# rlog58/dags-vae-search

Measured on AMD Instinct MI355X. Metric: DAGs/sec VAE+predictor train step, n=12 batch 4096 per GPU, at 1 MI355X, higher is better.
Workload: dtype f32 (fwd bf16x6, bwd bf16x3 split products, fp32 accumulate); 1 GPU; synthetic_v12 DAGs (n=12, card=12, N=15 tokens), PACE-VAE train step: pack + fwd + bwd + clip_grad_norm_(1.0) + Adam(1e-4), train mode dropout 0.15; per_gpu_batch=4096, global_batch=4096, waves_per_workgroup=8, parallelism=single

## Files before the change

### dags_vae_search_amd/csrc/dvs_api_backward.inc

```

static AttnBwdArgs attn_bwd_args(const Step& c, const DvsAttnP& ap, int block, int in, const DvsNormP* norm, const float* kv,
                                 const float* gpre, int site0) {
    AttnBwdArgs a;
    memset(&a, 0, sizeof(a));
    a.wimg = wimg_attn(c, block);
    a.dims = c.d;
    a.rec = c.rec;
    a.xin = c.ws + c.W.act[in];
    a.ln = ln_of(c, in, norm);
    a.kv = kv;
    a.in_w = c.P + ap.in_w;
    a.in_b = c.P + ap.in_b;
    a.out_w = c.P + ap.out_w;
    a.out_b = c.P + ap.out_b;
    a.gpre = gpre;
    a.gq = c.ws + c.W.gq;
    a.gk = c.ws + c.W.gk;
    a.gv = c.ws + c.W.gv;
    a.site_prob = site0;
    a.site_post = site0 + 1;
    a.slab = c.ws + c.W.slabs;
    a.P = c.L.total;
    a.o_out_w = ap.out_w;
    a.o_out_b = ap.out_b;
// ... 77 lines not shown
    const Step c = make_step(s, records, params, workspace, stream);
    if (int e = check_buffers(c, "dvs_loss_backward", records_bytes, n_params, workspace_bytes)) return e;
    const bool emit_loss = losses != nullptr;
    if (emit_loss && c.wide) return fail(13, "dvs_loss_backward_emit: one-tile path only (n_tokens, n_classes <= 16)");
    if (clip_scratch && 2 + dvs_sq_parts(c.L.total) > DVS_CLIP_SCRATCH_FLOATS)
        return fail(14, "dvs_loss_backward_sq: clip_scratch (DVS_CLIP_SCRATCH_FLOATS) is too small for this parameter count");
    call_begin();
    const DvsLayout& L = c.L;
    const DvsWorkspace& W = c.W;
    float* ws = c.ws;
    dvs_stream_t st = c.st;
    const bool wide = c.wide;
    const int grid = c.slabs;
    const int nw = c.nw;
    const bool chain = !wide && !split_stack();
    const bool chain_local = wide && !split_stack();
    BwdStackArgs stack;
    memset(&stack, 0, sizeof(stack));
    int stack_tag = 0;
    auto flush_stack = [&]() {
        if (stack.nphase > 0) dvs_launch_bwd_stack(stack, stack_tag, grid, nw, st);
        stack.nphase = 0;
        stack.has_latent = 0;
    };
    auto next_phase = [&](int kind) -> BwdPhase& {
        if (stack.nphase == DVS_STACK_PHASES) flush_stack();
        BwdPhase& ph = stack.ph[stack.nphase++];
        ph.kind = kind;
        return ph;
    };
    auto launch_ffn_bwd = [&](const FfnBwdArgs& f) {
        if (chain || chain_local) next_phase(DVS_PH_FFN).u.f = f;
        else dvs_launch_ffn_bwd(f, grid, nw, st);
    };
    auto launch_attn_bwd = [&](const AttnBwdArgs& a) {
        if (chain) {
            next_phase(DVS_PH_ATTN).u.a = a;
        } else if (wide) {
            flush_stack();
            dvs_launch_attn_bwd_w(a, grid, st);
        } else {
            dvs_launch_attn_bwd(a, grid, nw, st);
        }
    };
    auto launch_proj_bwd = [&](const ProjBwdArgs& a) {
        if (chain || chain_local) next_phase(DVS_PH_PROJ1 + 2).u.p = a;
        else dvs_launch_proj_bwd(a, 3, grid, nw, st);
    };

    float* cur = ws + W.gA;
    float* oth = ws + W.gB;
    {
        LossArgs la = loss_args(c);
        la.gcoef = gcoef;
        la.gout = cur;
        la.slab = ws + W.slabs;
        la.P = L.total;
        la.o_node0_w = L.node0_w;
        la.o_node0_b = L.node0_b;
        la.o_node2_w = L.node2_w;
        la.o_node2_b = L.node2_b;
        la.o_edge0_w = L.edge0_w;
        la.o_edge0_b = L.edge0_b;
        la.o_edge2_w = L.edge2_w;
        la.o_edge2_b = L.edge2_b;
        la.o_ln_g = L.dec[DVS_LAYERS - 1].n3.w;
        la.o_ln_b = L.dec[DVS_LAYERS - 1].n3.b;
        if (wide) dvs_launch_loss_bwd_w(la, grid, st);
        else dvs_launch_loss_bwd(la, grid, emit_loss, st);
        if (emit_loss) dvs_launch_finalize(finalize_args(c, status, losses, host_tail, host_seq), st);
    }
    const int dec_in = c.d.drop.on ? 7 : 0;
    for (int i = DVS_LAYERS - 1; i >= 0; --i) {
        const auto& pl = L.dec[i];
        const int s0 = slot_dec(i, 0), s1 = slot_dec(i, 1);
        launch_ffn_bwd(ffn_bwd_args(c, pl.ff, blk_dec_ffn(i), s1, pl.n2, cur, oth, site_dec(i, 4)));
        std::swap(cur, oth);
        launch_attn_bwd(attn_bwd_args(c, pl.ca, blk_dec_cross(i), s0, &pl.n1, ws + W.mem, cur, site_dec(i, 2)));
        ProjBwdArgs pq = proj_bwd_args(c, pl.ca, blk_dec_cross(i), s0, &pl.n1, cur, oth);
        pq.xin2 = ws + W.mem;
        pq.gout2 = ws + W.gmem;
        pq.accumulate_out2 = i != DVS_LAYERS - 1;
        launch_proj_bwd(pq);
        std::swap(cur, oth);
        const int sp = i > 0 ? slot_dec(i - 1, 2) : dec_in;
        const DvsNormP* np = i > 0 ? &L.dec[i - 1].n3 : nullptr;
        launch_attn_bwd(attn_bwd_args(c, pl.sa, blk_dec_self(i), sp, np, nullptr, cur, site_dec(i, 0)));
        launch_proj_bwd(proj_bwd_args(c, pl.sa, blk_dec_self(i), sp, np, cur, oth));
        std::swap(cur, oth);
    }
    flush_stack();
    stack_tag = 1;
    float* gdec_emb = cur;
    float* freebuf = oth;

    const bool fc_deferred = latent_in_chain(chain, nw);
    FcDwArgs fcdw;
    {
        LatentBwdArgs a;
        memset(&a, 0, sizeof(a));
        a.dims = c.d;
        a.gmem = ws + W.gmem;
        a.mu = ws + W.mu;
        a.logvar = ws + W.logvar;
        a.epsv = ws + W.epsv;
        a.limg = ws + W.limg;
        a.gcoef = gcoef;
        a.gz = ws + W.gz;
        a.genc = ws + W.genc;
        if (fc_deferred) {
            stack.has_latent = 1;
            stack.lat = a;
        } else {
            dvs_launch_latent_bwd(a, st);
        }
        FcDwArgs& f = fcdw;
        memset(&f, 0, sizeof(f));
        f.dims = c.d;
        f.gz = ws + W.gz;
        f.xenc = ws + W.enc_out;
        f.gmem = ws + W.gmem;
        f.z = ws + W.z;
        f.fcpart = ws + W.fcpart;
        f.P = L.total;
        f.o_fc1_w = L.fc1_w;
        f.o_fc1_b = L.fc1_b;
        f.o_fc2_w = L.fc2_w;
        f.o_fc2_b = L.fc2_b;
        f.o_fc3_w = L.fc3_w;
        f.o_fc3_b = L.fc3_b;
        if (!fc_deferred) dvs_launch_fc_dw(f, st);
    }
    cur = ws + W.genc;
    oth = freebuf;
    for (int i = DVS_LAYERS - 1; i >= 0; --i) {
        const auto& pl = L.enc[i];
        const int s0 = slot_enc(i, 0), s1 = slot_enc(i, 1);
        FfnBwdArgs f = ffn_bwd_args(c, pl.ff, blk_enc_ffn(i), s0, pl.n1, cur, oth, site_enc(i, 2));
        if (i == DVS_LAYERS - 1) {
            f.own_pre = ws + W.act[s1];
            f.own = ln_of(c, s1, &pl.n2);
            f.o_own_g = pl.n2.w;
            f.o_own_b = pl.n2.b;
        }
        launch_ffn_bwd(f);
        std::swap(cur, oth);
        const int sp = i > 0 ? slot_enc(i - 1, 1) : 0;
        const DvsNormP* np = i > 0 ? &L.enc[i - 1].n2 : nullptr;
        launch_attn_bwd(attn_bwd_args(c, pl.sa, blk_enc_attn(i), sp, np, nullptr, cur, site_enc(i, 0)));
        launch_proj_bwd(proj_bwd_args(c, pl.sa, blk_enc_attn(i), sp, np, cur, oth));
        std::swap(cur, oth);
    }
    flush_stack();
    if (fc_deferred) dvs_launch_fc_dw(fcdw, st);
    {
        EmbedArgs e = embed_args(c, 0);
        e.gout = cur;
        e.slab = ws + W.slabs;
        e.P = L.total;
        e.oW1 = L.W1;
        e.oW2 = L.W2;
        e.olab_w = L.lab_w;
        e.olab_b = L.lab_b;
        if (wide) dvs_launch_embed_bwd_w(e, gdec_emb, 2, grid, st);
        else dvs_launch_embed_bwd(e, gdec_emb, 2, grid, nw, st);
    }
    ReduceArgs r;
    r.slab = ws + W.slabs;
    r.fcpart = ws + W.fcpart;
    r.grads = grads;
    r.P = L.total;
    r.nslab = grid;
    r.fc_lo1 = L.fc1_w;
    r.fc_hi1 = L.dec[0].sa.in_w;
    r.fc_lo2 = L.fc3_w;
    r.fc_hi2 = L.total;
    r.sqpart = clip_scratch ? clip_scratch + 2 : nullptr;
    dvs_launch_reduce_slabs(r, st);
    return call_end("dvs_loss_backward");
}

extern "C" int dvs_clip_adam(int64_t n, float* params, float* grads, float* exp_avg, float* exp_avg_sq, float lr,
                             float beta1, float beta2, float adam_eps, int64_t step, float max_norm, float* scratch,
                             const float* guard, void* stream) {
    if (n <= 0 || !params || !grads || !exp_avg || !exp_avg_sq || !scratch) return fail(10, "dvs_clip_adam: bad argument");
    if (step < 1) return fail(12, "dvs_clip_adam: step is 1-based");
    call_begin();
    dvs_launch_clip_adam(n, params, grads, exp_avg, exp_avg_sq, lr, beta1, beta2, adam_eps, step, max_norm, scratch, guard, false,
                         (dvs_stream_t)stream);
    return call_end("dvs_clip_adam");
}

extern "C" int dvs_clip_adam_from_partials(int64_t n, float* params, float* grads, float* exp_avg, float* exp_avg_sq, float lr,
                                           float beta1, float beta2, float adam_eps, int64_t step, float max_norm,
                                           float* scratch, const float* guard, void* stream) {
    if (n <= 0 || !params || !grads || !exp_avg || !exp_avg_sq || !scratch) return fail(10, "dvs_clip_adam_from_partials: bad argument");
    if (step < 1) return fail(12, "dvs_clip_adam_from_partials: step is 1-based");
    if (2 + dvs_sq_parts(n) > DVS_CLIP_SCRATCH_FLOATS) return fail(14, "dvs_clip_adam_from_partials: more partials than the scratch holds");
    call_begin();
    dvs_launch_clip_adam(n, params, grads, exp_avg, exp_avg_sq, lr, beta1, beta2, adam_eps, step, max_norm, scratch, guard, true,
                         (dvs_stream_t)stream);
    return call_end("dvs_clip_adam_from_partials");
}
```

### dags_vae_search_amd/csrc/dvs_backward.h

```cpp
#pragma once
#include "dvs_kernels.h"
#include "dvs_stage.h"

struct FfnBwdArgs {
    DvsDims dims;
    const float* xin;
    DvsLN ln;
    const float *l1_w, *l1_b, *l2_w, *l2_b;
    const void* wimg;
    const float* gpre;
    const float* own_pre;
    DvsLN own;
    float* gout;
    int site_hidden, site_post;
    float* slab;
    int64_t P;
    int64_t o_l1_w, o_l1_b, o_l2_w, o_l2_b, o_ln_g, o_ln_b, o_own_g, o_own_b;
};

struct ProjBwdArgs {
    DvsDims dims;
    const float* xin;
    DvsLN ln;
    const float* w;
    const void* wimg;
    const float* gy[3];
    const float* gres;
    float* gout;
    int accumulate_out;
    int slot_order;
    const float* xin2;
    float* gout2;
    int accumulate_out2;
    float* slab;
    int64_t P;
    int64_t o_w, o_b, o_ln_g, o_ln_b;
};

struct AttnBwdArgs {
    DvsDims dims;
    const DvsRecord* rec;
    const float* xin;
    DvsLN ln;
    const float* kv;
    const float *in_w, *in_b, *out_w, *out_b;
    const void* wimg;
    const float* gpre;
    float *gq, *gk, *gv;
    int site_prob, site_post;
    float* slab;
    int64_t P;
    int64_t o_out_w, o_out_b;
    const float* qkv;
};

struct LatentBwdArgs {
    DvsDims dims;
    const float* gmem;
    const float *mu, *logvar, *epsv;
    const float* limg;
    const float* gcoef;
    float* gz;
    float* genc;
};

struct FcDwArgs {
    DvsDims dims;
    const float* gz;
    const float* xenc;
    const float* gmem;
    const float* z;
    float* fcpart;
    int64_t P;
    int64_t o_fc1_w, o_fc1_b, o_fc2_w, o_fc2_b, o_fc3_w, o_fc3_b;
};

struct ReduceArgs {
    const float* slab;
    const float* fcpart;
    float* grads;
    int64_t P;
    int nslab;
    int64_t fc_lo1, fc_hi1, fc_lo2, fc_hi2;
    float* sqpart;
};

enum { DVS_PH_FFN = 0, DVS_PH_ATTN = 1, DVS_PH_PROJ1 = 2, DVS_PH_PROJ2 = 3, DVS_PH_PROJ3 = 4 };
#define DVS_STACK_PHASES 9
struct BwdPhase {
    int kind, pad;
    union {
        FfnBwdArgs f;
        AttnBwdArgs a;
        ProjBwdArgs p;
    } u;
};
struct BwdStackArgs {
    int nphase;
    int has_latent;
    BwdPhase ph[DVS_STACK_PHASES];
    DvsStagePlan plan[DVS_STACK_PHASES];
    LatentBwdArgs lat;
};
static_assert(sizeof(BwdStackArgs) <= 4096, "kernel argument block limit");
void dvs_launch_bwd_stack(const BwdStackArgs& s, int tag, int grid, int nw, dvs_stream_t st);
void dvs_launch_ffn_bwd(const FfnBwdArgs& a, int grid, int nw, dvs_stream_t st);
void dvs_launch_proj_bwd(const ProjBwdArgs& a, int nproj, int grid, int nw, dvs_stream_t st);
void dvs_launch_attn_bwd(const AttnBwdArgs& a, int grid, int nw, dvs_stream_t st);
void dvs_launch_loss_bwd(const LossArgs& a, int grid, bool emit_loss, dvs_stream_t st);
void dvs_launch_embed_bwd(const EmbedArgs& a, const float* gout2, int site2, int grid, int nw, dvs_stream_t st);
void dvs_launch_latent_bwd(const LatentBwdArgs& a, dvs_stream_t st);
void dvs_launch_fc_dw(const FcDwArgs& a, dvs_stream_t st);
void dvs_launch_reduce_slabs(const ReduceArgs& a, dvs_stream_t st);
void dvs_launch_clip_adam(int64_t n, float* params, float* grads, float* m, float* v, float lr, float b1, float b2,
                          float eps, int64_t step, float max_norm, float* scratch, const float* guard, bool have_partials,
                          dvs_stream_t st);
inline int dvs_sq_parts(int64_t n) { return (int)(((n + 3) / 4 + 63) / 64); }

template <int OT, int IT>
__device__ __forceinline__ void dvs_stage_dw(float* region, const f4 (&dw)[OT][IT], const Lane& L) {
    constexpr int COLS = 16 * IT;
    float* mine = region + L.wave * (256 * OT * IT);
#pragma unroll
    for (int ot = 0; ot < OT; ++ot)
#pragma unroll
        for (int it = 0; it < IT; ++it)
#pragma unroll
            for (int reg = 0; reg < 4; ++reg) mine[(16 * ot + 4 * L.g + reg) * COLS + 16 * it + L.r] = dw[ot][it][reg];
}
template <int OT, int IT>
__device__ __forceinline__ void dvs_flush_dw(const float* region, float* dst, const Lane& L, int rows = 16 * OT,
                                             int ld_dst = 16 * IT, int cols_used = 16 * IT, bool rperm = false,
                                             bool cperm = false) {
    constexpr int COLS = 16 * IT, SZ = 256 * OT * IT;
    if (cperm) {
        for (int i = dvs_tid(); i < rows * COLS; i += blockDim.x) {
            float s = region[i];
            for (int w = 1; w < L.nwaves; ++w) s += region[w * SZ + i];
            const int row = i / COLS, col = i - row * COLS;
            dst[(size_t)(rperm ? dvs_pi(row) : row) * ld_dst + (cperm ? dvs_pi(col) : col)] = s;
        }
        return;
    }
    if (cols_used == COLS && (ld_dst & 3) == 0) {
        for (int i = dvs_tid() * 4; i < rows * COLS; i += blockDim.x * 4) {
            f4 s = *(const f4*)(region + i);
            for (int w = 1; w < L.nwaves; ++w) s += *(const f4*)(region + w * SZ + i);
            const int row = i / COLS, col = i - row * COLS;
            *(f4*)(dst + (size_t)(rperm ? dvs_pi(row) : row) * ld_dst + col) = s;
        }
        return;
    }
    for (int i = dvs_tid(); i < rows * COLS; i += blockDim.x) {
        float s = region[i];
        for (int w = 1; w < L.nwaves; ++w) s += region[w * SZ + i];
        const int row = i / COLS, col = i - row * COLS;
        if (col < cols_used) dst[(size_t)row * ld_dst + col] = s;
    }
}
template <int NT>
__device__ __forceinline__ void dvs_stage_vec(float* region, const f4 (&v)[NT], float* scr, const Lane& L) {
#pragma unroll
    for (int t = 0; t < NT; ++t) *(f4*)(scr + L.r * DVS_LD + 16 * t + 4 * L.g) = v[t];
    dvs_wave_sync();
    if (L.lane < 16 * NT) {
        float s = 0.f;
#pragma unroll
        for (int rr = 0; rr < 16; ++rr) s += scr[rr * DVS_LD + L.lane];
        region[L.wave * (16 * NT) + L.lane] = s;
    }
    dvs_wave_sync();
}
template <int NT>
__device__ __forceinline__ void dvs_flush_vec(const float* region, float* dst, const Lane& L, int n = 16 * NT,
                                              bool perm = false) {
    for (int i = dvs_tid(); i < n; i += blockDim.x) {
        float s = region[i];
        for (int w = 1; w < L.nwaves; ++w) s += region[w * (16 * NT) + i];
        dst[perm ? dvs_pi(i) : i] = s;
    }
}
constexpr int DVS_RED_MAT = 4 * 4096;
constexpr int DVS_RED_VEC = 4 * 64;

__device__ __forceinline__ void dvs_ln_bwd(f4 (&dx)[4], const f4 (&xhat)[4], float rstd, const float* lg, f4 (&dgam)[4],
                                           f4 (&dbet)[4], const Lane& L) {
    float s1 = 0.f, s2 = 0.f;
#pragma unroll
    for (int t = 0; t < 4; ++t) {
        const f4 g = dvs_vecT(lg, t, L);
#pragma unroll
        for (int kk = 0; kk < 4; ++kk) {
            dgam[t][kk] += dx[t][kk] * xhat[t][kk];
            dbet[t][kk] += dx[t][kk];
            const float dxh = dx[t][kk] * g[kk];
            dx[t][kk] = dxh;
            s1 += dxh;
            s2 += dxh * xhat[t][kk];
        }
    }
    s1 = dvs_sum_g(s1) * (1.f / 64.f);
    s2 = dvs_sum_g(s2) * (1.f / 64.f);
#pragma unroll
    for (int t = 0; t < 4; ++t)
#pragma unroll
        for (int kk = 0; kk < 4; ++kk) dx[t][kk] = rstd * (dx[t][kk] - s1 - xhat[t][kk] * s2);
}

struct DvsGroup {
    int* counter;
    int target;
};
__device__ __forceinline__ void dvs_group_barrier(DvsGroup& G, const Lane& L) {
    G.target += 4;
#ifdef DVS_EMU
    if (L.lane == 0) atomicAdd(G.counter, 1);
    while (__atomic_load_n(G.counter, __ATOMIC_RELAXED) < G.target) emu::yield();
    (void)emu::exchange(0, 0);
#else
    __builtin_amdgcn_fence(__ATOMIC_RELEASE, "workgroup");
    if (L.lane == 0) atomicAdd(G.counter, 1);
    for (int spins = 0; __hip_atomic_load(G.counter, __ATOMIC_RELAXED, __HIP_MEMORY_SCOPE_WORKGROUP) < G.target &&
                        spins < (1 << 24); ++spins)
        __builtin_amdgcn_s_sleep(1);
    __builtin_amdgcn_fence(__ATOMIC_ACQUIRE, "workgroup");
#endif
}
__device__ __forceinline__ void dvs_park_T(float* slot, const f4 (&v)[4], const Lane& L) {
#pragma unroll
    for (int t = 0; t < 4; ++t) *(f4*)(slot + L.r * DVS_LD + 16 * t + 4 * L.g) = v[t];
}
__device__ __forceinline__ float dvs_colsum(const float* slot, const Lane& L) {
    float s = 0.f;
#pragma unroll
    for (int rr = 0; rr < 16; ++rr) s += slot[rr * DVS_LD + L.lane];
    return s;
}
template <int NW = 8>
__device__ __forceinline__ void dvs_coop_stage(float* buf, const f4 (&acc)[4], const Lane& L) {
    if (NW == 4 || L.wave >= 4) return;
    const int ot = L.wave & 3;
#pragma unroll
    for (int it = 0; it < 4; ++it)
#pragma unroll
        for (int reg = 0; reg < 4; ++reg) buf[(16 * ot + 4 * L.g + reg) * 64 + 16 * it + L.r] = acc[it][reg];
}
template <int NW = 8>
__device__ __forceinline__ void dvs_coop_flush(const float* buf, float* dst, const f4 (&acc)[4], const Lane& L, bool rperm = false,
                                               bool cperm = false, int ld_dst = 64) {
    if (NW == 8 && L.wave < 4) return;
    const int ot = L.wave & 3;
#pragma unroll
    for (int it = 0; it < 4; ++it)
#pragma unroll
        for (int reg = 0; reg < 4; ++reg) {
            const int row = 16 * ot + 4 * L.g + reg, col = 16 * it + L.r;
            const float v = NW == 8 ? acc[it][reg] + buf[row * 64 + col] : acc[it][reg];
            dst[(size_t)(rperm ? dvs_pi(row) : row) * ld_dst + (cperm ? dvs_pi(col) : col)] = v;
        }
}
__device__ __forceinline__ void dvs_ln_bwd_core(f4 (&dx)[4], const f4 (&xhat)[4], float rstd, const float* lg, const Lane& L) {
    float s1 = 0.f, s2 = 0.f;
#pragma unroll
    for (int t = 0; t < 4; ++t) {
        const f4 g = dvs_vecT(lg, t, L);
// ... 24 lines not shown
```

### dags_vae_search_amd/csrc/k_backward_heads.hip

```cpp
#include "dvs_backward.h"
#include "dvs_wimg.h"
#include "dvs_latent_bwd.h"
#include "dvs_loss.h"

#ifdef DVS_STAMPS
__device__ unsigned long long dvs_stamps_lossb[256 * 4 * 12];
DVS_STAMP_READER(lossb)
#endif
#define LBSTAMP(k) DVS_ACC_STAMP_AT(dvs_stamps_lossb, lst_, 4, 12, k)
template <bool EMIT>
__global__ __launch_bounds__(256) void k_loss_bwd(LossArgs a, DvsStagePlan plan) {
#ifdef DVS_STAMPS
    unsigned long long lst_ = __builtin_amdgcn_s_memtime();
#endif
    DVS_DYN_LDS(smem);
    const LossLds l = loss_lds(smem);
    const int N = a.dims.N, C = a.dims.C;
    dvs_stage_now<(LOSS_CHUNKS + 3) / 4>(&plan, smem);
    __syncthreads();
    const Lane L = dvs_lane();
    float* scrV = l.scr + L.wave * 3 * DVS_SCR;
    float* scrU = scrV + DVS_SCR;
    float* dlm = scrU + DVS_SCR;
    const float b2 = l.b2[0];
// ... 108 lines not shown
            dvs_matb3<4>(V, hs, l.Wb, 64, 0, L);
        }
#pragma unroll
        for (int t = 0; t < 4; ++t) {
            *(f4*)(scrV + L.r * DVS_LD + 16 * t + 4 * L.g) = V[t];
            *(f4*)(scrU + L.r * DVS_LD + 16 * t + 4 * L.g) = U[t];
        }
        dvs_wave_sync();
        const unsigned par = rec->parents[(L.r + 1) & 15];
        LBSTAMP(3);
        f4 sU[4] = {f4_zero(), f4_zero(), f4_zero(), f4_zero()}, sV[4] = {f4_zero(), f4_zero(), f4_zero(), f4_zero()};
        for (int j0 = 0; j0 < N - 2; j0 += 2) {
            f4 pre[2][4], ev[2] = {f4_zero(), f4_zero()};
            const bool has2 = j0 + 1 < N - 2;
            const int jj[2] = {j0, has2 ? j0 + 1 : j0};
#pragma unroll
            for (int u = 0; u < 2; ++u)
#pragma unroll
                for (int t = 0; t < 4; ++t) {
                    const f4 x = U[t] + *(const f4*)(scrV + jj[u] * DVS_LD + 16 * t + 4 * L.g);
#pragma unroll
                    for (int kk = 0; kk < 4; ++kk) pre[u][t][kk] = fmaxf(x[kk], 0.f);
                    ev[u] += w2v[t] * pre[u][t];
                }
            float dl[2];
#pragma unroll
            for (int u = 0; u < 2; ++u) {
                const float logit = dvs_sum_g((ev[u][0] + ev[u][1]) + (ev[u][2] + ev[u][3])) + b2;
                const bool pv = (L.r > jj[u]) && (L.r <= N - 2) && (u == 0 || has2);
                const float truth = (float)((par >> (jj[u] + 1)) & 1u);
                const float sg = dvs_rcp(1.0f + __expf(-logit));
                dl[u] = pv ? gr * (sg - truth) : 0.f;
                if constexpr (EMIT) {
                    const float x = logit;
                    const float bce = fmaxf(x, 0.f) - x * truth + __logf(1.0f + __expf(-fabsf(x)));
                    enll += (pv && (jj[u] & 3) == L.g) ? bce : 0.f;
                }
            }
#pragma unroll
            for (int u = 0; u < 2; ++u)
#pragma unroll
                for (int t = 0; t < 4; ++t) {
                    dw2[t] += pre[u][t] * dl[u];
                    f4 st;
#pragma unroll
                    for (int kk = 0; kk < 4; ++kk) st[kk] = fminf(fmaxf(pre[u][t][kk] * 1.0e30f, 0.f), 1.f);
                    sU[t] += st * dl[u];
                }
            if (L.g == 0) {
                db2 += dl[0] + dl[1];
                dlm[L.r * 16 + j0] = dl[0];
                if (has2) dlm[L.r * 16 + j0 + 1] = dl[1];
            }
        }
        dvs_wave_sync();
        LBSTAMP(4);
#pragma unroll 2
        for (int i = 1; i <= N - 2; ++i) {
            const float dl = (L.r < i) ? dlm[i * 16 + L.r] : 0.f;
#pragma unroll
            for (int t = 0; t < 4; ++t) {
                const f4 x = *(const f4*)(scrU + i * DVS_LD + 16 * t + 4 * L.g) + V[t];
                f4 st;
#pragma unroll
                for (int kk = 0; kk < 4; ++kk) st[kk] = fminf(fmaxf(x[kk] * 1.0e30f, 0.f), 1.f);
                sV[t] += st * dl;
            }
        }
#pragma unroll
        for (int t = 0; t < 4; ++t) {
            dU[t] = w2v[t] * sU[t];
            dV[t] = w2v[t] * sV[t];
        }
        dvs_wave_sync();
        LBSTAMP(5);
        dvs_park_bf((dvs_bf16*)scrV, dU, L);
        dvs_park_bf((dvs_bf16*)scrU, dV, L);
        dvs_park_bf((dvs_bf16*)dlm, h, L);
        __syncthreads();
        dvs_coop_dw_bf(aWa, abU, slots, slots + 2 * 2 * DVS_SCR, SLOT_STRIDE, L);
        dvs_coop_dw_bf(aWb, abV, slots + 2 * DVS_SCR, slots + 2 * 2 * DVS_SCR, SLOT_STRIDE, L);
        __syncthreads();
        LBSTAMP(6);
        dvs_matb_T<4>(dh, dvs_split_T(dU), l.WaT, l.WaT + DVS_IMG64, 0, L);
        dvs_matb_T<4>(dh, dvs_split_T(dV), l.WbT, l.WbT + DVS_IMG64, 0, L);
        dvs_ln_bwd(dh, xhat, rstd, l.lg, dgam, dbet, L);
        dvs_store_tile(a.gout, dag, dh, L);
        if constexpr (EMIT) {
            nll += enll;
            nll = dvs_sum_wave(nll);
            if (L.lane == 0) a.dag_loss[(size_t)dag * 2] = nll;
        }
#ifndef DVS_EMU
        asm volatile("" ::"v"(touch));
#else
        (void)touch;
#endif
        LBSTAMP(7);
    }
    __syncthreads();
    LBSTAMP(8);
    float* slab = a.slab + (size_t)blockIdx.x * a.P;
    {
        dvs_coop_flush<4>(nullptr, slab + a.o_edge0_w, aWa, L, false, false, 128);
        dvs_coop_flush<4>(nullptr, slab + a.o_edge0_w + 64, aWb, L, false, false, 128);
        if (L.r == 0) {
#pragma unroll
            for (int reg = 0; reg < 4; ++reg) slab[a.o_edge0_b + 16 * L.wave + 4 * L.g + reg] = abV[reg];
        }
        float* rN1 = (float*)smem;
        float* rN2 = rN1 + 4 * 2048;
        float* rv = rN2 + 4 * 512;
        dvs_stage_dw<2, 4>(rN1, dWn1, L);
        dvs_stage_dw<1, 2>(rN2, dWn2, L);
        float* es = rv + 192 + 4 * DVS_RED_VEC + 16 + L.wave * DVS_SCR;
        dvs_stage_vec<2>(rv, dbn1, es, L);
        dvs_stage_vec<1>(rv + 128, dbn2, es, L);
        dvs_stage_vec<4>(rv + 192 + DVS_RED_VEC, dw2, es, L);
        dvs_stage_vec<4>(rv + 192 + 2 * DVS_RED_VEC, dgam, es, L);
        dvs_stage_vec<4>(rv + 192 + 3 * DVS_RED_VEC, dbet, es, L);
        const float sb2 = dvs_sum_wave(L.g == 0 ? db2 : 0.f);
        float* rb2 = rv + 192 + 4 * DVS_RED_VEC;
        if (L.lane == 0) rb2[L.wave] = sb2;
        __syncthreads();
        dvs_flush_dw<2, 4>(rN1, slab + a.o_node0_w, L);
        dvs_flush_dw<1, 2>(rN2, slab + a.o_node2_w, L, C, 32);
        dvs_flush_vec<2>(rv, slab + a.o_node0_b, L);
        dvs_flush_vec<1>(rv + 128, slab + a.o_node2_b, L, C);
        dvs_flush_vec<4>(rv + 192 + DVS_RED_VEC, slab + a.o_edge2_w, L);
        dvs_flush_vec<4>(rv + 192 + 2 * DVS_RED_VEC, slab + a.o_ln_g, L);
        dvs_flush_vec<4>(rv + 192 + 3 * DVS_RED_VEC, slab + a.o_ln_b, L);
        if (threadIdx.x == 0) {
            float s = rb2[0];
            for (int w = 1; w < L.nwaves; ++w) s += rb2[w];
            slab[a.o_edge2_b] = s;
        }
    }
    LBSTAMP(9);
}

void dvs_launch_loss_bwd(const LossArgs& a, int grid, bool emit_loss, dvs_stream_t st) {
    const size_t lds = loss_lds_bytes(4, 3);
    DvsStagePlan plan;
    loss_plan(plan, a);
    if (emit_loss) {
        DVS_SET_LDS(k_loss_bwd<true>, lds);
        DVS_LAUNCH_AS("k_loss_bwd", k_loss_bwd<true>, dim3(grid), dim3(256), lds, st, a, plan);
    } else {
        DVS_SET_LDS(k_loss_bwd<false>, lds);
        DVS_LAUNCH_AS("k_loss_bwd", k_loss_bwd<false>, dim3(grid), dim3(256), lds, st, a, plan);
    }
}

__global__ __launch_bounds__(512) void k_embed_bwd(EmbedArgs a, const float* gout2, int site2, DvsStagePlan plan) {
    DVS_DYN_LDS(smem);
    const int N = a.dims.N, C = a.dims.C;
    float* W1 = (float*)smem;
    float* W2 = W1 + 2 * DVS_MAXTOK * DVS_LD;
    float* labw = W2 + 64 * EMB_LDW2;
    float* labb = labw + 32 * 16;
    float* scr0 = labb + 32;
    if (blockDim.x >= 512) dvs_stage_now<3>(&plan, smem);
    else dvs_stage_now<5>(&plan, smem);
    __syncthreads();
    const Lane L = dvs_lane();
    const DvsDrop D = dvs_drop_of(a.dims);
    float* scr = scr0 + L.wave * DVS_SCR;
    f4 dW2[4][2], dlabb[2], dW1a[1][4], dW1b[1][4], dlab[2][1];
#pragma unroll
    for (int i = 0; i < 4; ++i) dW2[i][0] = dW2[i][1] = dW1a[0][i] = dW1b[0][i] = f4_zero();
    dlabb[0] = dlabb[1] = dlab[0][0] = dlab[1][0] = f4_zero();
    for (int dag = blockIdx.x * L.nwaves + L.wave; dag < a.dims.B; dag += gridDim.x * L.nwaves) {
        const DvsRecord* rec = a.rec + dag;
        const bool valid = L.r < N;
        const int label = rec->label[L.r];
        const uint32_t gdag = a.dims.dag_offset + dag;
        const EmbSel sel = dvs_emb_selectors(rec, N, scr, L);
        f4 e1[4];
        dvs_emb_hidden(e1, W1, N, sel, L);
        for (int src = 0; src < 2; ++src) {
            const float* gsrc = src == 0 ? a.gout : gout2;
            if (!gsrc) continue;
            const int site = src == 0 ? a.site : site2;
            f4 gx[4];
            dvs_load_grad(gx, gsrc, dag, N, L);
            f4 dle[2];
#pragma unroll
            for (int t = 0; t < 2; ++t)
#pragma unroll
                for (int kk = 0; kk < 4; ++kk) {
                    const int f = 16 * t + 4 * L.g + kk;
                    const float pre = labw[f * 16 + label] + labb[f];
                    dle[t][kk] = (valid && pre > 0.f) ? gx[t][kk] : 0.f;
                }
            dlabb[0] += dle[0];
            dlabb[1] += dle[1];
            const uint32_t k1 = dvs_site_key(a.dims.seed_lo, a.dims.seed_hi, site, gdag);
            f4 m1[4] = {f4_splat(1.f), f4_splat(1.f), f4_splat(1.f), f4_splat(1.f)};
            dvs_dropout_tile(m1, k1, D, L);
            f4 e1d[4];
#pragma unroll
            for (int t = 0; t < 4; ++t) e1d[t] = e1[t] * m1[t];
            f4 de2[2] = {gx[2], gx[3]};
            dvs_dropout_tile<2>(de2, dvs_site_key(a.dims.seed_lo, a.dims.seed_hi, site + 1, gdag), D, L);
            f4 e1dN[4], de2N[2], dleN[2];
            dvs_t2n<4>(e1dN, e1d, scr, L);
            dvs_t2n<2>(de2N, de2, scr, L);
            dvs_t2n<2>(dleN, dle, scr, L);
            dvs_outer_acc<4, 2>(dW2, e1dN, de2N);
            f4 de1[4] = {f4_zero(), f4_zero(), f4_zero(), f4_zero()};
            dvs_mat_T<4, 2>(de1, de2, W2, EMB_LDW2, 0, L);
#pragma unroll
            for (int t = 0; t < 4; ++t) de1[t] *= m1[t];
#pragma unroll
            for (int t = 0; t < 4; ++t)
#pragma unroll
                for (int kk = 0; kk < 4; ++kk) de1[t][kk] = e1[t][kk] > 0.f ? de1[t][kk] : 0.f;
            f4 de1N[4];
            dvs_t2n<4>(de1N, de1, scr, L);
            f4 selA[1] = {sel.selA}, parA[1] = {sel.parA}, labA[1] = {sel.labA};
            dvs_outer_acc<1, 4>(dW1a, selA, de1N);
            dvs_outer_acc<1, 4>(dW1b, parA, de1N);
            dvs_outer_acc<2, 1>(dlab, dleN, labA);
        }
    }
    __syncthreads();
    float* slab = a.slab + (size_t)blockIdx.x * a.P;
    float* r1a = (float*)smem;
    float* r1b = r1a + 8 * 1024;
    float* rlab = r1b + 8 * 1024;
    float* rv = rlab + 8 * 512;
    dvs_stage_dw<1, 4>(r1a, dW1a, L);
    dvs_stage_dw<1, 4>(r1b, dW1b, L);
    dvs_stage_dw<2, 1>(rlab, dlab, L);
    dvs_stage_vec<2>(rv, dlabb, rv + 8 * 32 + L.wave * DVS_SCR, L);
    __syncthreads();
    dvs_flush_dw<1, 4>(r1a, slab + a.oW1, L, N, 64);
    dvs_flush_dw<1, 4>(r1b, slab + a.oW1 + (size_t)N * 64, L, N, 64);
    dvs_flush_dw<2, 1>(rlab, slab + a.olab_w, L, 32, C, C);
    dvs_flush_vec<2>(rv, slab + a.olab_b, L);
    __syncthreads();
    float* rW2 = (float*)smem;
    dvs_stage_dw<4, 2>(rW2, dW2, L);
    __syncthreads();
    dvs_flush_dw<4, 2>(rW2, slab + a.oW2, L);
}

void dvs_launch_embed_bwd(const EmbedArgs& a, const float* gout2, int site2, int grid, int nw, dvs_stream_t st) {
    size_t lds = (2 * DVS_MAXTOK * DVS_LD + 64 * EMB_LDW2 + 32 * 16 + 32 + 8 * DVS_SCR) * 4;
    const size_t red = (8 * (1024 + 1024 + 512) + 8 * 32 + 8 * DVS_SCR) * 4;
    if (lds < red) lds = red;
    DvsStagePlan plan;
    dvs_plan_clear(plan);
    dvs_plan_seg(plan, DVS_FAKE_LDS, DVS_FAKE_LDS, a.embimg, 2 * DvsEmbImg::FLOATS);
    dvs_plan_seal(plan);
    DVS_SET_LDS(k_embed_bwd, lds);
    DVS_LAUNCH(k_embed_bwd, dim3(grid), dim3(nw == 4 ? 256 : 512), lds, st, a, gout2, site2, plan);
}

constexpr int LATB_WAVES = 8;
__global__ __launch_bounds__(64 * LATB_WAVES) void k_latent_bwd(LatentBwdArgs a) {
    __shared__ f4 part[LATB_WAVES][2][64];
    dvs_latent_bwd_group<LATB_WAVES>(a, part, (int)blockIdx.x * 16, (int)blockIdx.x * 16 + 8);
}

void dvs_launch_latent_bwd(const LatentBwdArgs& a, dvs_stream_t st) {
    const int ngroups = (a.dims.B + 15) / 16;
    DVS_LAUNCH(k_latent_bwd, dim3(ngroups), dim3(64 * LATB_WAVES), 0, st, a);
}

constexpr int FC_MT = 4;
__global__ __launch_bounds__(512) void k_fc_dw(FcDwArgs a) {
    __shared__ f4 red[4][FC_MT * 6 + 2][64];
    const Lane L = dvs_lane();
    const int B = a.dims.B, N = a.dims.N;
    const int ldw = N * 64;
    const int nmg = 16 * a.dims.NT;
    const int mg = blockIdx.x % nmg, q = blockIdx.x / nmg;
    const size_t dstride = (size_t)a.dims.NT * DVS_TILE;
    const int per_q = (B + DVS_FC_PARTS - 1) / DVS_FC_PARTS;
    const int per_w = (per_q + 7) / 8;
    const int d0 = q * per_q + L.wave * per_w;
    int d1 = d0 + per_w;
    if (d1 > (q + 1) * per_q) d1 = (q + 1) * per_q;
    if (d1 > B) d1 = B;
    f4 acc[FC_MT][4], acc3[FC_MT][2];
    f4 bs3 = f4_zero();
    f4 bsfc = f4_zero();
#pragma unroll
    for (int j = 0; j < FC_MT; ++j) {
#pragma unroll
        for (int t = 0; t < 4; ++t) acc[j][t] = f4_zero();
        acc3[j][0] = acc3[j][1] = f4_zero();
    }
    for (int c0 = d0; c0 < d1; c0 += 16) {
        float ga[4][4], zb[4][2], xb[4][FC_MT], gm[4][FC_MT], live[4];
#pragma unroll
        for (int ks = 0; ks < 4; ++ks) {
            const int d = c0 + 4 * ks + L.g;
            const bool dv = d < d1;
            const size_t dd = dv ? d : 0;
            live[ks] = dv ? 1.f : 0.f;
#pragma unroll
            for (int t = 0; t < 4; ++t) ga[ks][t] = a.gz[dd * 64 + 16 * t + L.r];
#pragma unroll
            for (int t = 0; t < 2; ++t) zb[ks][t] = a.z[dd * 32 + 16 * t + L.r];
#pragma unroll
            for (int j = 0; j < FC_MT; ++j) {
                xb[ks][j] = a.xenc[dd * dstride + 16 * (FC_MT * mg + j) + L.r];
                gm[ks][j] = a.gmem[dd * dstride + 16 * (FC_MT * mg + j) + L.r];
            }
        }
#pragma unroll
        for (int ks = 0; ks < 4; ++ks) {
#pragma unroll
            for (int t = 0; t < 4; ++t) ga[ks][t] *= live[ks];
#pragma unroll
            for (int j = 0; j < FC_MT; ++j) {
                gm[ks][j] *= live[ks];
                bs3[j] += gm[ks][j];
            }
#pragma unroll
            for (int t = 0; t < 4; ++t) bsfc[t] += ga[ks][t];
#pragma unroll
            for (int j = 0; j < FC_MT; ++j) {
#pragma unroll
                for (int t = 0; t < 4; ++t) acc[j][t] = dvs_mfma(ga[ks][t], xb[ks][j], acc[j][t]);
#pragma unroll
                for (int t = 0; t < 2; ++t) acc3[j][t] = dvs_mfma(gm[ks][j], zb[ks][t], acc3[j][t]);
            }
        }
    }
#pragma unroll
    for (int j = 0; j < FC_MT; ++j) bs3[j] = dvs_sum_g(bs3[j]);
#pragma unroll
    for (int t = 0; t < 4; ++t) bsfc[t] = dvs_sum_g(bsfc[t]);
    if (L.wave < 4) {
#pragma unroll
        for (int j = 0; j < FC_MT; ++j) {
#pragma unroll
            for (int t = 0; t < 4; ++t) red[L.wave][6 * j + t][L.lane] = acc[j][t];
            red[L.wave][6 * j + 4][L.lane] = acc3[j][0];
            red[L.wave][6 * j + 5][L.lane] = acc3[j][1];
        }
        red[L.wave][6 * FC_MT][L.lane] = bsfc;
        red[L.wave][6 * FC_MT + 1][L.lane] = bs3;
    }
    __syncthreads();
    if (L.wave >= 4) {
        const int w = L.wave - 4;
#pragma unroll
        for (int j = 0; j < FC_MT; ++j) {
#pragma unroll
            for (int t = 0; t < 4; ++t) red[w][6 * j + t][L.lane] += acc[j][t];
            red[w][6 * j + 4][L.lane] += acc3[j][0];
            red[w][6 * j + 5][L.lane] += acc3[j][1];
        }
        red[w][6 * FC_MT][L.lane] += bsfc;
        red[w][6 * FC_MT + 1][L.lane] += bs3;
    }
    __syncthreads();
    if (L.wave >= 4) return;
    const int j = L.wave;
    const int m = FC_MT * mg + j;
    f4 tot[8];
#pragma unroll
    for (int i = 0; i < 6; ++i) {
        tot[i] = red[0][6 * j + i][L.lane];
#pragma unroll
        for (int w = 1; w < 4; ++w) tot[i] += red[w][6 * j + i][L.lane];
    }
#pragma unroll
    for (int i = 0; i < 2; ++i) {
        tot[6 + i] = red[0][6 * FC_MT + i][L.lane];
#pragma unroll
        for (int w = 1; w < 4; ++w) tot[6 + i] += red[w][6 * FC_MT + i][L.lane];
    }
    float* out = a.fcpart + (size_t)q * a.P;
    const int mm = m & 63;
    {
        const int tok = 16 * (m >> 6) + 4 * (mm & 3) + (L.r >> 2);
        const int f = 16 * (mm >> 4) + 4 * ((mm >> 2) & 3) + (L.r & 3);
        if (tok < N) {
#pragma unroll
            for (int t = 0; t < 4; ++t)
#pragma unroll
                for (int reg = 0; reg < 4; ++reg) {
                    const int o = 16 * (t & 1) + 4 * L.g + reg;
                    out[(t < 2 ? a.o_fc1_w : a.o_fc2_w) + (size_t)o * ldw + tok * 64 + f] = tot[t][reg];
                }
            if (L.g == 0) {
                const float b3 = j == 0 ? tot[7][0] : j == 1 ? tot[7][1] : j == 2 ? tot[7][2] : tot[7][3];
                out[a.o_fc3_b + tok * 64 + f] = b3;
            }
        }
    }
    {
        const int tok = 16 * (m >> 6) + 4 * (mm & 3) + L.g;
        const int fb = 16 * (mm >> 4) + 4 * ((mm >> 2) & 3);
        if (tok < N) {
#pragma unroll
            for (int t = 0; t < 2; ++t)
#pragma unroll
                for (int reg = 0; reg < 4; ++reg)
                    out[a.o_fc3_w + (size_t)(tok * 64 + fb + reg) * 32 + 16 * t + L.r] = tot[4 + t][reg];
        }
    }
    if (mg == 0 && j == 0 && L.g == 0) {
#pragma unroll
        for (int t = 0; t < 4; ++t) out[(t < 2 ? a.o_fc1_b : a.o_fc2_b) + 16 * (t & 1) + L.r] = tot[6][t];
    }
}

void dvs_launch_fc_dw(const FcDwArgs& a, dvs_stream_t st) {
    DVS_LAUNCH(k_fc_dw, dim3(16 * a.dims.NT * DVS_FC_PARTS), dim3(512), 0, st, a);
}
```

### dags_vae_search_amd/csrc/k_optim.hip

```cpp
#include "dvs_backward.h"

constexpr int SQ_PARTS = 256;
__global__ __launch_bounds__(256) void k_sqnorm_part(const float* g, int64_t n, float* scratch) {
    __shared__ float part[256];
    float s = 0.f;
    const int64_t n4 = n >> 2;
    for (int64_t i = (int64_t)blockIdx.x * 256 + threadIdx.x; i < n4; i += (int64_t)SQ_PARTS * 256) {
        const f4 v = *(const f4*)(g + 4 * i);
        s += (v[0] * v[0] + v[1] * v[1]) + (v[2] * v[2] + v[3] * v[3]);
    }
    if (blockIdx.x == 0)
        for (int64_t i = 4 * n4 + threadIdx.x; i < n; i += 256) s += g[i] * g[i];
    part[threadIdx.x] = s;
    __syncthreads();
    for (int k = 128; k > 0; k >>= 1) {
        if ((int)threadIdx.x < k) part[threadIdx.x] += part[threadIdx.x + k];
        __syncthreads();
    }
    if (threadIdx.x == 0) scratch[2 + blockIdx.x] = part[0];
}
__global__ __launch_bounds__(256) void k_adam(int64_t n, float* p, float* g, float* m, float* v, float lr, float b1, float b2,
                                              float eps, float bc1, float bc2_sqrt, float max_norm, float* scratch,
                                              const float* guard, int nparts) {
    __shared__ float part[256];
    {
        float s = 0.f;
        for (int i = threadIdx.x; i < nparts; i += 256) s += scratch[2 + i];
        part[threadIdx.x] = s;
    }
    __syncthreads();
    for (int k = 128; k > 0; k >>= 1) {
        if ((int)threadIdx.x < k) part[threadIdx.x] += part[threadIdx.x + k];
        __syncthreads();
    }
    const float ss = part[0];
    float coef = 1.0f;
    if (max_norm > 0.f) {
        coef = max_norm / (sqrtf(ss) + 1e-6f);
        coef = coef < 1.0f ? coef : 1.0f;
    }
    if (blockIdx.x == 0 && threadIdx.x == 0) {
        scratch[0] = ss;
        scratch[1] = coef;
    }
    if (guard && (guard[0] != 0.f || guard[1] != 0.f)) return;
    const int64_t i = (int64_t)blockIdx.x * blockDim.x + threadIdx.x;
    if (i >= n) return;
    const float gi = g[i] * coef;
    g[i] = gi;
    const float mi = b1 * m[i] + (1.0f - b1) * gi;
    const float vi = b2 * v[i] + (1.0f - b2) * gi * gi;
    m[i] = mi;
    v[i] = vi;
    const float denom = sqrtf(vi) / bc2_sqrt + eps;
    p[i] -= (lr / bc1) * (mi / denom);
}

void dvs_launch_clip_adam(int64_t n, float* params, float* grads, float* m, float* v, float lr, float b1, float b2,
                          float eps, int64_t step, float max_norm, float* scratch, const float* guard, bool have_partials,
                          dvs_stream_t st) {
    if (!have_partials) DVS_LAUNCH(k_sqnorm_part, dim3(SQ_PARTS), dim3(256), 0, st, (const float*)grads, n, scratch);
    const float bc1 = 1.0f - powf(b1, (float)step);
    const float bc2 = 1.0f - powf(b2, (float)step);
    DVS_LAUNCH(k_adam, dim3((unsigned)((n + 255) / 256)), dim3(256), 0, st, n, params, grads, m, v, lr, b1, b2, eps,
                       bc1, sqrtf(bc2), max_norm, scratch, guard, have_partials ? dvs_sq_parts(n) : SQ_PARTS);
}

#include "dvs_wimg.h"
__device__ __forceinline__ float dvs_loss_head_value(const DvsLossHeadArgs& h, int i) {
    if (i < 32 * 68) {
        const int r = i / 68, c = i % 68;
        return c < 64 ? h.node0_w[r * 64 + c] : 0.f;
    }
    i -= 32 * 68;
    if (i < 16 * 36) {
        const int c = i / 36, k = i % 36;
        return (c < h.C && k < 32) ? h.node2_w[c * 32 + k] : 0.f;
    }
    i -= 16 * 36;
    if (i < 32) return h.node0_b[i];
    i -= 32;
    if (i < 16) return i < h.C ? h.node2_b[i] : 0.f;
    i -= 16;
    if (i < 64) return h.edge0_b[i];
    i -= 64;
    if (i < 64) return h.edge2_w[i];
    i -= 64;
    if (i < 16) return i == 0 ? h.edge2_b[0] : 0.f;
    i -= 16;
    if (i < 64) return h.ln_g[i];
    return h.ln_b[i - 64];
}
__device__ __forceinline__ float dvs_emb_block_value(const DvsLossHeadArgs& h, int i) {
    if (i < 32 * 68) {
        const int r = i / 68, c = i % 68;
        return (r < 2 * h.N && c < 64) ? h.W1[r * 64 + c] : 0.f;
    }
    i -= 32 * 68;
    if (i < 64 * 36) {
        const int f = i / 36, k = i % 36;
        return k < 32 ? h.W2[f * 32 + k] : 0.f;
    }
    i -= 64 * 36;
    if (i < 512) {
        const int f = i >> 4, c = i & 15;
        return c < h.C ? h.lab_w[f * h.C + c] : 0.f;
    }
    i -= 512;
    return i < 32 ? h.lab_b[i] : 0.f;
}
__global__ __launch_bounds__(256) void k_prepare_images(DvsImgJobs jobs, const float* params, dvs_bf16* wimg, DvsLatImgArgs lat,
                                                        DvsLossHeadArgs head) {
    const int nlat = 1024 * lat.NT / 64;
    const int first_job = nlat + (head.dst ? 2 : 0);
    if (head.dst) {
        if ((int)blockIdx.x == nlat + 1) {
            float v[DvsEmbImg::FLOATS / 256];
#pragma unroll
            for (int u = 0; u < DvsEmbImg::FLOATS / 256; ++u) v[u] = dvs_emb_block_value(head, u * 256 + (int)threadIdx.x);
#pragma unroll
            for (int u = 0; u < DvsEmbImg::FLOATS / 256; ++u) head.dst_emb[u * 256 + threadIdx.x] = v[u];
            return;
        }
        if ((int)blockIdx.x == nlat) {
            float v[DvsLossImg::HEAD_FLOATS / 256];
#pragma unroll
            for (int u = 0; u < DvsLossImg::HEAD_FLOATS / 256; ++u) v[u] = dvs_loss_head_value(head, u * 256 + (int)threadIdx.x);
#pragma unroll
            for (int u = 0; u < DvsLossImg::HEAD_FLOATS / 256; ++u) head.dst[u * 256 + threadIdx.x] = v[u];
            return;
        }
    }
    if ((int)blockIdx.x < nlat) {
        __shared__ float tile[64][65];
        const int K = 1024 * lat.NT, kp0 = (int)blockIdx.x * 64;
        const int l = threadIdx.x & 63, w = threadIdx.x >> 6;
        const size_t ldw = (size_t)lat.N * 64;
        auto col_of = [&](int kp, bool& valid) {
            const int tile_i = kp >> 10, q = (kp & 1023) >> 2, kk = kp & 3, t = q >> 6, ln = q & 63;
            const int tok = 16 * tile_i + (ln & 15), feat = 16 * t + 4 * (ln >> 4) + kk;
            valid = tok < lat.N;
            return (size_t)(valid ? tok : 0) * 64 + feat;
        };
        bool valid;
        const size_t col = col_of(kp0 + l, valid);
        float va[16];
#pragma unroll
        for (int i = 0; i < 16; ++i) {
            const int o = w + 4 * i;
            va[i] = !valid ? 0.f : (o < 32 ? lat.fc1_w[o * ldw + col] : lat.fc2_w[(o - 32) * ldw + col]);
        }
        float v3[8];
#pragma unroll
        for (int i = 0; i < 8; ++i) {
            bool v2;
            const size_t c2 = col_of(kp0 + 2 * (w + 4 * i) + (l >> 5), v2);
            v3[i] = v2 ? lat.fc3_w[c2 * 32 + (l & 31)] : 0.f;
        }
        const float vb3 = valid ? lat.fc3_b[col] : 0.f;
#pragma unroll
        for (int i = 0; i < 16; ++i) {
            const int o = w + 4 * i;
            tile[o][l] = va[i];
            lat.img[DvsLatImg::A(lat.NT) + (size_t)o * DvsLatImg::LD(lat.NT) + kp0 + l] = va[i];
        }
        __syncthreads();
        for (int j = w; j < 64; j += 4) lat.img[DvsLatImg::AT(lat.NT) + (size_t)(kp0 + j) * 64 + l] = tile[l][j];
        __syncthreads();
#pragma unroll
        for (int i = 0; i < 8; ++i) {
            const int jj = 2 * (w + 4 * i) + (l >> 5), o = l & 31;
            tile[o][jj] = v3[i];
            lat.img[DvsLatImg::W3(lat.NT) + (size_t)(kp0 + jj) * 32 + o] = v3[i];
        }
        __syncthreads();
        for (int o = w; o < 32; o += 4) lat.img[DvsLatImg::W3T(lat.NT) + (size_t)o * DvsLatImg::LD(lat.NT) + kp0 + l] = tile[o][l];
        if (w == 0) lat.img[DvsLatImg::B3(lat.NT) + kp0 + l] = vb3;
        return;
    }
    const int jb = ((int)blockIdx.x - first_job) / 12, slice = ((int)blockIdx.x - first_job) % 12;
// ... 30 lines not shown
```

Baseline: 3.505 million DAGs/s.

## Fuse deferred fc weight-gradient kernel into embed backward launch and prefetch fc operands

The deferred fc dW kernel no longer runs as its own launch after the backward stack. It now shares one grid with the embed backward kernel: the first blocks compute fc dW and the remaining blocks do embed backward, which removes a launch and lets the two independent jobs run at the same time. The fc dW loop now software-pipelines its global loads one round ahead, using a sched barrier. The clip partial-sum read is unrolled into independent loads. The shared LDS size becomes the larger of the two needs, which may cut occupancy for the embed blocks, and the fused path forces 512-thread blocks.

```diff
diff --git a/dags_vae_search_amd/csrc/dvs_api_backward.inc b/dags_vae_search_amd/csrc/dvs_api_backward.inc
--- a/dags_vae_search_amd/csrc/dvs_api_backward.inc
+++ b/dags_vae_search_amd/csrc/dvs_api_backward.inc
@@ -253,7 +253,6 @@
         std::swap(cur, oth);
     }
     flush_stack();
-    if (fc_deferred) dvs_launch_fc_dw(fcdw, st);
     {
         EmbedArgs e = embed_args(c, 0);
         e.gout = cur;
@@ -264,6 +263,7 @@
         e.olab_w = L.lab_w;
         e.olab_b = L.lab_b;
         if (wide) dvs_launch_embed_bwd_w(e, gdec_emb, 2, grid, st);
+        else if (fc_deferred) dvs_launch_embed_fc_bwd(e, gdec_emb, 2, grid, fcdw, st);
         else dvs_launch_embed_bwd(e, gdec_emb, 2, grid, nw, st);
     }
     ReduceArgs r;
diff --git a/dags_vae_search_amd/csrc/dvs_backward.h b/dags_vae_search_amd/csrc/dvs_backward.h
--- a/dags_vae_search_amd/csrc/dvs_backward.h
+++ b/dags_vae_search_amd/csrc/dvs_backward.h
@@ -111,6 +111,7 @@
 void dvs_launch_embed_bwd(const EmbedArgs& a, const float* gout2, int site2, int grid, int nw, dvs_stream_t st);
 void dvs_launch_latent_bwd(const LatentBwdArgs& a, dvs_stream_t st);
 void dvs_launch_fc_dw(const FcDwArgs& a, dvs_stream_t st);
+void dvs_launch_embed_fc_bwd(const EmbedArgs& a, const float* gout2, int site2, int grid, const FcDwArgs& fc, dvs_stream_t st);
 void dvs_launch_reduce_slabs(const ReduceArgs& a, dvs_stream_t st);
 void dvs_launch_clip_adam(int64_t n, float* params, float* grads, float* m, float* v, float lr, float b1, float b2,
                           float eps, int64_t step, float max_norm, float* scratch, const float* guard, bool have_partials,
diff --git a/dags_vae_search_amd/csrc/k_backward_heads.hip b/dags_vae_search_amd/csrc/k_backward_heads.hip
--- a/dags_vae_search_amd/csrc/k_backward_heads.hip
+++ b/dags_vae_search_amd/csrc/k_backward_heads.hip
@@ -284,8 +284,8 @@
     }
 }
 
-__global__ __launch_bounds__(512) void k_embed_bwd(EmbedArgs a, const float* gout2, int site2, DvsStagePlan plan) {
-    DVS_DYN_LDS(smem);
+__device__ __forceinline__ void dvs_embed_bwd_block(const EmbedArgs& a, const float* gout2, int site2, const DvsStagePlan& plan,
+                                                    char* smem, int bid, int nblk) {
     const int N = a.dims.N, C = a.dims.C;
     float* W1 = (float*)smem;
     float* W2 = W1 + 2 * DVS_MAXTOK * DVS_LD;
@@ -302,7 +302,7 @@
 #pragma unroll
     for (int i = 0; i < 4; ++i) dW2[i][0] = dW2[i][1] = dW1a[0][i] = dW1b[0][i] = f4_zero();
     dlabb[0] = dlabb[1] = dlab[0][0] = dlab[1][0] = f4_zero();
-    for (int dag = blockIdx.x * L.nwaves + L.wave; dag < a.dims.B; dag += gridDim.x * L.nwaves) {
+    for (int dag = bid * L.nwaves + L.wave; dag < a.dims.B; dag += nblk * L.nwaves) {
         const DvsRecord* rec = a.rec + dag;
         const bool valid = L.r < N;
         const int label = rec->label[L.r];
@@ -357,7 +357,7 @@
         }
     }
     __syncthreads();
-    float* slab = a.slab + (size_t)blockIdx.x * a.P;
+    float* slab = a.slab + (size_t)bid * a.P;
     float* r1a = (float*)smem;
     float* r1b = r1a + 8 * 1024;
     float* rlab = r1b + 8 * 1024;
@@ -378,14 +378,26 @@
     dvs_flush_dw<4, 2>(rW2, slab + a.oW2, L);
 }
 
-void dvs_launch_embed_bwd(const EmbedArgs& a, const float* gout2, int site2, int grid, int nw, dvs_stream_t st) {
+__global__ __launch_bounds__(512) void k_embed_bwd(EmbedArgs a, const float* gout2, int site2, DvsStagePlan plan) {
+    DVS_DYN_LDS(smem);
+    dvs_embed_bwd_block(a, gout2, site2, plan, smem, (int)blockIdx.x, (int)gridDim.x);
+}
+
+static size_t embed_bwd_lds_bytes() {
     size_t lds = (2 * DVS_MAXTOK * DVS_LD + 64 * EMB_LDW2 + 32 * 16 + 32 + 8 * DVS_SCR) * 4;
     const size_t red = (8 * (1024 + 1024 + 512) + 8 * 32 + 8 * DVS_SCR) * 4;
-    if (lds < red) lds = red;
-    DvsStagePlan plan;
+    return lds < red ? red : lds;
+}
+static void embed_bwd_plan(DvsStagePlan& plan, const EmbedArgs& a) {
     dvs_plan_clear(plan);
     dvs_plan_seg(plan, DVS_FAKE_LDS, DVS_FAKE_LDS, a.embimg, 2 * DvsEmbImg::FLOATS);
     dvs_plan_seal(plan);
+}
+
+void dvs_launch_embed_bwd(const EmbedArgs& a, const float* gout2, int site2, int grid, int nw, dvs_stream_t st) {
+    const size_t lds = embed_bwd_lds_bytes();
+    DvsStagePlan plan;
+    embed_bwd_plan(plan, a);
     DVS_SET_LDS(k_embed_bwd, lds);
     DVS_LAUNCH(k_embed_bwd, dim3(grid), dim3(nw == 4 ? 256 : 512), lds, st, a, gout2, site2, plan);
 }
@@ -402,13 +414,38 @@
 }
 
 constexpr int FC_MT = 4;
-__global__ __launch_bounds__(512) void k_fc_dw(FcDwArgs a) {
-    __shared__ f4 red[4][FC_MT * 6 + 2][64];
+constexpr int FC_ROWS = FC_MT * 6 + 2;
+typedef f4 (*FcRed)[FC_ROWS][64];
+
+struct FcRound {
+    float ga[4][4], zb[4][2], xb[4][FC_MT], gm[4][FC_MT], live[4];
+};
+
+__device__ __forceinline__ void dvs_fc_load(FcRound& o, const FcDwArgs& a, int c0, int d1, int mg, size_t dstride, const Lane& L) {
+#pragma unroll
+    for (int ks = 0; ks < 4; ++ks) {
+        const int d = c0 + 4 * ks + L.g;
+        const bool dv = d < d1;
+        const size_t dd = dv ? d : 0;
+        o.live[ks] = dv ? 1.f : 0.f;
+#pragma unroll
+        for (int t = 0; t < 4; ++t) o.ga[ks][t] = a.gz[dd * 64 + 16 * t + L.r];
+#pragma unroll
+        for (int t = 0; t < 2; ++t) o.zb[ks][t] = a.z[dd * 32 + 16 * t + L.r];
+#pragma unroll
+        for (int j = 0; j < FC_MT; ++j) {
+            o.xb[ks][j] = a.xenc[dd * dstride + 16 * (FC_MT * mg + j) + L.r];
+            o.gm[ks][j] = a.gmem[dd * dstride + 16 * (FC_MT * mg + j) + L.r];
+        }
+    }
+}
+
+__device__ __forceinline__ void dvs_fc_dw_block(const FcDwArgs& a, FcRed red, int bid) {
     const Lane L = dvs_lane();
     const int B = a.dims.B, N = a.dims.N;
     const int ldw = N * 64;
     const int nmg = 16 * a.dims.NT;
-    const int mg = blockIdx.x % nmg, q = blockIdx.x / nmg;
+    const int mg = bid % nmg, q = bid / nmg;
     const size_t dstride = (size_t)a.dims.NT * DVS_TILE;
     const int per_q = (B + DVS_FC_PARTS - 1) / DVS_FC_PARTS;
     const int per_w = (per_q + 7) / 8;
@@ -425,41 +462,31 @@
         for (int t = 0; t < 4; ++t) acc[j][t] = f4_zero();
         acc3[j][0] = acc3[j][1] = f4_zero();
     }
+    FcRound nxt;
+    dvs_fc_load(nxt, a, d0, d1, mg, dstride, L);
     for (int c0 = d0; c0 < d1; c0 += 16) {
-        float ga[4][4], zb[4][2], xb[4][FC_MT], gm[4][FC_MT], live[4];
+        FcRound o = nxt;
+        if (c0 + 16 < d1) dvs_fc_load(nxt, a, c0 + 16, d1, mg, dstride, L);
+#ifndef DVS_EMU
+        __builtin_amdgcn_sched_barrier(0);
+#endif
 #pragma unroll
         for (int ks = 0; ks < 4; ++ks) {
-            const int d = c0 + 4 * ks + L.g;
-            const bool dv = d < d1;
-            const size_t dd = dv ? d : 0;
-            live[ks] = dv ? 1.f : 0.f;
-#pragma unroll
-            for (int t = 0; t < 4; ++t) ga[ks][t] = a.gz[dd * 64 + 16 * t + L.r];
-#pragma unroll
-            for (int t = 0; t < 2; ++t) zb[ks][t] = a.z[dd * 32 + 16 * t + L.r];
+#pragma unroll
+            for (int t = 0; t < 4; ++t) o.ga[ks][t] *= o.live[ks];
 #pragma unroll
             for (int j = 0; j < FC_MT; ++j) {
-                xb[ks][j] = a.xenc[dd * dstride + 16 * (FC_MT * mg + j) + L.r];
-                gm[ks][j] = a.gmem[dd * dstride + 16 * (FC_MT * mg + j) + L.r];
-            }
-        }
-#pragma unroll
-        for (int ks = 0; ks < 4; ++ks) {
-#pragma unroll
-            for (int t = 0; t < 4; ++t) ga[ks][t] *= live[ks];
+                o.gm[ks][j] *= o.live[ks];
+                bs3[j] += o.gm[ks][j];
+            }
+#pragma unroll
+            for (int t = 0; t < 4; ++t) bsfc[t] += o.ga[ks][t];
 #pragma unroll
             for (int j = 0; j < FC_MT; ++j) {
-                gm[ks][j] *= live[ks];
-                bs3[j] += gm[ks][j];
-            }
-#pragma unroll
-            for (int t = 0; t < 4; ++t) bsfc[t] += ga[ks][t];
-#pragma unroll
-            for (int j = 0; j < FC_MT; ++j) {
-#pragma unroll
-                for (int t = 0; t < 4; ++t) acc[j][t] = dvs_mfma(ga[ks][t], xb[ks][j], acc[j][t]);
-#pragma unroll
-                for (int t = 0; t < 2; ++t) acc3[j][t] = dvs_mfma(gm[ks][j], zb[ks][t], acc3[j][t]);
+#pragma unroll
+                for (int t = 0; t < 4; ++t) acc[j][t] = dvs_mfma(o.ga[ks][t], o.xb[ks][j], acc[j][t]);
+#pragma unroll
+                for (int t = 0; t < 2; ++t) acc3[j][t] = dvs_mfma(o.gm[ks][j], o.zb[ks][t], acc3[j][t]);
             }
         }
     }
@@ -544,6 +571,31 @@
     }
 }
 
+__global__ __launch_bounds__(512) void k_fc_dw(FcDwArgs a) {
+    __shared__ f4 red[4][FC_ROWS][64];
+    dvs_fc_dw_block(a, red, (int)blockIdx.x);
+}
+
 void dvs_launch_fc_dw(const FcDwArgs& a, dvs_stream_t st) {
     DVS_LAUNCH(k_fc_dw, dim3(16 * a.dims.NT * DVS_FC_PARTS), dim3(512), 0, st, a);
 }
+
+__global__ __launch_bounds__(512) void k_embed_fc_bwd(EmbedArgs a, const float* gout2, int site2, DvsStagePlan plan, FcDwArgs fc,
+                                                      int nfc) {
+    DVS_DYN_LDS(smem);
+    if ((int)blockIdx.x < nfc) {
+        dvs_fc_dw_block(fc, (FcRed)smem, (int)blockIdx.x);
+        return;
+    }
+    dvs_embed_bwd_block(a, gout2, site2, plan, smem, (int)blockIdx.x - nfc, (int)gridDim.x - nfc);
+}
+
+void dvs_launch_embed_fc_bwd(const EmbedArgs& a, const float* gout2, int site2, int grid, const FcDwArgs& fc, dvs_stream_t st) {
+    size_t lds = embed_bwd_lds_bytes();
+    if (lds < sizeof(f4) * 4 * FC_ROWS * 64) lds = sizeof(f4) * 4 * FC_ROWS * 64;
+    const int nfc = 16 * fc.dims.NT * DVS_FC_PARTS;
+    DvsStagePlan plan;
+    embed_bwd_plan(plan, a);
+    DVS_SET_LDS(k_embed_fc_bwd, lds);
+    DVS_LAUNCH(k_embed_fc_bwd, dim3(nfc + grid), dim3(512), lds, st, a, gout2, site2, plan, fc, nfc);
+}
diff --git a/dags_vae_search_amd/csrc/k_optim.hip b/dags_vae_search_amd/csrc/k_optim.hip
--- a/dags_vae_search_amd/csrc/k_optim.hip
+++ b/dags_vae_search_amd/csrc/k_optim.hip
@@ -24,8 +24,17 @@
                                               const float* guard, int nparts) {
     __shared__ float part[256];
     {
+        constexpr int MAXR = (DVS_CLIP_SCRATCH_FLOATS - 2 + 255) / 256;
+        float v[MAXR];
+#pragma unroll
+        for (int u = 0; u < MAXR; ++u) {
+            const int i = (int)threadIdx.x + u * 256;
+            v[u] = i < nparts ? scratch[2 + i] : 0.f;
+        }
         float s = 0.f;
-        for (int i = threadIdx.x; i < nparts; i += 256) s += scratch[2 + i];
+#pragma unroll
+        for (int u = 0; u < MAXR; ++u)
+            if ((int)threadIdx.x + u * 256 < nparts) s += v[u];
         part[threadIdx.x] = s;
     }
     __syncthreads();
```

Measured after the change: 3.521 million DAGs/s (median of 6 runs). No clear change (+0.5%).
